# DCMMC/halo2-scaffold

Measured on AMD Instinct MI355X. Metric: create_proof() wall-clock + MSM G1-adds/s at k=20 standard_plonk, 1/2/4/8 GPU, higher is better.
Workload: dtype u32 (254-bit Montgomery integers as 9 x 29-bit limbs, 64-bit multiply-accumulate); 1 GPU; standard_plonk hot-path replay k=20: 11 MSM(2^20) + 6 iNTT(2^20) + 6 coset-NTT(2^21) + 1 coset-iNTT(2^21); k=20, scalar_distribution=uniform, msm_window_bits=17, msm_windows=15, msm_buckets=65536, parallelism=single-gpu, deployment=one process, one GPU, combine=none (single GPU)

## Files before the change

halo2-scaffold_amd/csrc/h2mi_msm.hip:

```cpp

#include <algorithm>
#include <map>
#include <vector>

#include "g1.cuh"
#include "g1_29.cuh"
#include "g1_29_quad.cuh"
#include "h2mi_internal.h"
#include "scan.cuh"

namespace h2 {

constexpr uint32_t S0_MAX = 128;
constexpr uint32_t S1 = 8;
constexpr uint32_t FG_NARROW = 8;
constexpr uint32_t FG_WIDE = 2;
constexpr size_t SHIFT_MIN_N = 4096;
constexpr uint32_t HOT_MIN = 64;
constexpr uint32_t HOT_MIN_WIDE = 8;

constexpr uint32_t ACCUM_RESIDENT_CHUNKS = 256 * 2 * 256;
__host__ __device__ inline uint32_t accum_rounds(uint32_t entries) {
  const uint32_t per_round = S0_MAX * ACCUM_RESIDENT_CHUNKS;
  return entries ? (entries + per_round - 1) / per_round : 1;
}
constexpr uint32_t ACCUM_GATHER_ONLY_MAX = 16384;
__host__ __device__ inline uint32_t accum_chunk_len(uint32_t entries) {
  if (entries <= ACCUM_GATHER_ONLY_MAX) return 1;
  const uint32_t slots = accum_rounds(entries) * ACCUM_RESIDENT_CHUNKS;
  const uint32_t s0 = (entries + slots - 1) / slots;
  return s0 < 8 ? 8 : s0;
}

struct Slot {
  uint32_t* vals[2] = {nullptr, nullptr};
  uint8_t* bkeys = nullptr;
  uint32_t* bincnt = nullptr;
  uint32_t* binbase = nullptr;
  uint32_t* binseg = nullptr;
  uint32_t* tile_live = nullptr;
  uint32_t* off = nullptr;
  uint32_t* s0_dev = nullptr;
  uint32_t* np[2] = {nullptr, nullptr};
  uint32_t* toff[2] = {nullptr, nullptr};
  uint8_t* part[2] = {nullptr, nullptr};
  uint8_t* dense = nullptr;
  uint8_t *dense2 = nullptr, *vsum = nullptr;
  uint32_t* tseg[2] = {nullptr, nullptr};
  uint8_t* rc = nullptr;
  uint8_t* g = nullptr;
  uint64_t* stats = nullptr;
  fe* shift = nullptr;
  hipEvent_t input_ready = nullptr, head_done = nullptr, accum_done = nullptr, tail_done = nullptr;
  bool tail_pending = false, accum_pending = false, head_pending = false;
  bool tail_ever = false, accum_ever = false, head_ever = false;
  hipStream_t last_stream = nullptr;
  bool tail_deferred = false;
  void* d_out = nullptr;
  uint32_t tasks1 = 0;
  uint8_t* sdig = nullptr;
  uint8_t* spart = nullptr;
  uint32_t* scnt = nullptr;
  bool small_deferred = false;
  uint32_t small_n = 0;
};
constexpr int NSLOT = 8;

struct Bases {
  int dev = 0;
  size_t n = 0;
  size_t stride = 0;
  bool has_sum = false;
// ... 95 lines not shown

template <uint32_t CT, class F>
__device__ __forceinline__ void for_each_digit(const fe& s, uint32_t c_rt, uint32_t W_rt, F&& f) {
  const uint32_t c = CT ? CT : c_rt;
  const uint32_t W = CT ? (255 + CT - 1) / CT : W_rt;
  uint32_t carry = 0;
  const uint32_t half = 1u << (c - 1);
#pragma unroll
  for (uint32_t w = 0; w < W; w++) {
    uint32_t bit = w * c;
    uint32_t limb = bit >> 5, sh = bit & 31;
    uint32_t raw = 0;
    if (limb < 8) {
      uint64_t two = s.v[limb];
      if (limb + 1 < 8) two |= (uint64_t)s.v[limb + 1] << 32;
      raw = (uint32_t)(two >> sh) & ((1u << c) - 1);
    }
    uint32_t d = raw + carry;
    uint32_t mag = d, neg = 0;
    carry = 0;
    if (d > half) {
      mag = (1u << c) - d;
      neg = 1;
      carry = 1;
    }
    if (mag) f(w, mag - 1, neg);
  }
}


__device__ __forceinline__ void msm_pick_shift_body(const fe* scalars, size_t n, fe* shift_out) {
  __shared__ fe smp[64];
  const uint32_t lane = threadIdx.x;
  size_t idx = (n / 64) * lane + n / 128;
  if (idx >= n) idx = n - 1;
  const fe v = fe_load(&scalars[idx]);
  smp[lane] = v;
  __syncthreads();
  uint32_t same = 0;
  for (uint32_t j = 0; j < 64; j++) same += fe_eq(v, smp[j]) ? 1u : 0u;
  const uint64_t winners = __ballot(same >= 40);
  if (lane == 0) fe_store(shift_out, winners ? smp[__ffsll((unsigned long long)winners) - 1] : fe_zero());
}
__global__ void __launch_bounds__(64) k_msm_pick_shift(const fe* scalars, size_t n, fe* shift_out) { msm_pick_shift_body(scalars, n, shift_out); }
__device__ __forceinline__ fe msm_scalar(const fe* scalars, size_t i, size_t n, const fe* shift) {
  fe x;
  if (!shift) {
    x = fe_load(&scalars[i]);
  } else {
    const fe v = fe_load(shift);
    x = i < n ? fe_sub<FrP>(fe_load(&scalars[i]), v) : v;
  }
  if (fe_is_zero(x)) return x;
  f29 c = f29_zero();
  c.v[0] = 32;
  fe o;
  f29_pack(f29_reduce_canonical<Fr29>(f29_mul<Fr29>(f29_unpack(x.v), c)), o.v);
  return o;
}

template <uint32_t CT>
__device__ __forceinline__ void msm_bin_count_body(const fe* scalars, size_t n, const fe* shift, uint32_t c, uint32_t W, uint32_t lb, uint32_t nbins,
                                                   uint32_t ntiles, uint32_t* cnt_out, uint32_t* tile_live) {
  __shared__ uint32_t cnt[NBINS_MAX];
  __shared__ uint32_t any_live;
  const uint32_t tid = threadIdx.x;
  if (tid < NBINS_MAX) cnt[tid] = 0;
  if (tid == 0) any_live = 0;
  __syncthreads();
  size_t i = (size_t)blockIdx.x * P1_TS + tid;
  if (i < n + (shift ? 1 : 0)) {
    fe s = msm_scalar(scalars, i, n, shift);
    if (!fe_is_zero(s)) {
      any_live = 1;
      for_each_digit<CT>(s, c, W, [&](uint32_t, uint32_t bucket, uint32_t) { atomicAdd(&cnt[bin_of<(CT >= WIDE_MIN_C)>(bucket, lb)], 1u); });
    }
  }
  __syncthreads();
  if (tid == 0) tile_live[blockIdx.x] = any_live;
  if (tid < nbins) cnt_out[(size_t)tid * ntiles + blockIdx.x] = cnt[tid];
  if (blockIdx.x == 0 && tid == 0) cnt_out[(size_t)nbins * ntiles] = 0;
}
template <uint32_t CT>
__global__ void __launch_bounds__(P1_TS) k_msm_bin_count(const fe* scalars, size_t n, const fe* shift, uint32_t c, uint32_t W, uint32_t lb,
                                                         uint32_t nbins, uint32_t ntiles, uint32_t* cnt_out, uint32_t* tile_live) {
  msm_bin_count_body<CT>(scalars, n, shift, c, W, lb, nbins, ntiles, cnt_out, tile_live);
}

extern __shared__ uint4 h2_msm_smem[];

template <uint32_t CT>
__device__ __forceinline__ void msm_bin_scatter_body(const fe* scalars, size_t n, const fe* shift, size_t n_reg, uint32_t c, uint32_t W, uint32_t lb,
                                                     uint32_t nbins, uint32_t ntiles, const uint32_t* base, uint32_t* vals_out, void* keys_out_,
                                                     const uint32_t* tile_live) {
  constexpr bool WIDE = CT >= WIDE_MIN_C;
  if (!tile_live[blockIdx.x]) return;
  __shared__ uint32_t cnt[NBINS_MAX], lstart[NBINS_MAX + 1], wsum[NBINS_MAX / 64];
  uint32_t* stage_val = reinterpret_cast<uint32_t*>(h2_msm_smem);
  uint16_t* stage_key = reinterpret_cast<uint16_t*>(stage_val + P1_TS * W);
  const uint32_t tid = threadIdx.x, lane = tid & 63, wave = tid >> 6, tile = blockIdx.x;
  uint32_t gb = 0;
  if (tid < NBINS_MAX) {
    cnt[tid] = 0;
    gb = tid < nbins ? base[(size_t)tid * ntiles + tile] : 0;
  }
  __syncthreads();
  size_t i = (size_t)tile * P1_TS + tid;
  fe s;
  const bool live = i < n + (shift ? 1 : 0);
  constexpr uint32_t WK = CT ? (255 + CT - 1) / CT : 1;
  uint32_t ent[WK], rk[WK];
#pragma unroll
  for (uint32_t w = 0; w < WK; w++) ent[w] = 0xFFFFFFFFu;
  bool live_nz = false;
  if (live) {
    s = msm_scalar(scalars, i, n, shift);
    live_nz = !fe_is_zero(s);
  }
  if (live_nz) {
// ... 43 lines not shown
  __syncthreads();
  const uint32_t total = lstart[NBINS_MAX];
  if (WIDE) {
    uint16_t* keys_out = reinterpret_cast<uint16_t*>(keys_out_);
    for (uint32_t p = tid; p < total; p += P1_TS) {
      uint32_t lo = 0, hi = NBINS_MAX;
      while (hi - lo > 1) {
        const uint32_t mid = (lo + hi) >> 1;
        if (lstart[mid] <= p) lo = mid;
        else hi = mid;
      }
      const uint32_t dst = p + cnt[lo];
      vals_out[dst] = stage_val[p];
      keys_out[dst] = stage_key[p];
    }
  } else {
    uint8_t* keys_out = reinterpret_cast<uint8_t*>(keys_out_);
    for (uint32_t p = tid; p < total; p += P1_TS) {
      const uint32_t key = stage_key[p];
      const uint32_t dst = p + cnt[key >> lb];
      vals_out[dst] = stage_val[p];
      keys_out[dst] = (uint8_t)(key & mask);
    }
  }
}
template <uint32_t CT>
__global__ void __launch_bounds__(P1_TS) k_msm_bin_scatter(const fe* scalars, size_t n, const fe* shift, size_t n_reg, uint32_t c, uint32_t W,
                                                           uint32_t lb, uint32_t nbins, uint32_t ntiles, const uint32_t* base, uint32_t* vals_out,
                                                           void* keys_out_, const uint32_t* tile_live) {
  msm_bin_scatter_body<CT>(scalars, n, shift, n_reg, c, W, lb, nbins, ntiles, base, vals_out, keys_out_, tile_live);
}

constexpr uint32_t NQ_MAX = 128;
__device__ __forceinline__ void msm_bin_sort_body(const uint8_t* keys_in, const uint32_t* vals_in, const uint32_t* base, uint32_t ntiles, uint32_t nbins,
                                                  uint32_t lb, uint32_t s0_fixed, uint32_t nb, uint32_t* vals_out, uint32_t* off, uint32_t* np0,
                                                  uint32_t* np1, uint32_t* s0_out) {
  __shared__ uint32_t wh[P2_THREADS / 64][NQ_MAX];
  __shared__ uint32_t run[NQ_MAX], ccnt[NQ_MAX], cstart[NQ_MAX], carry64;
  __shared__ uint32_t stage[P2_CH];
  __shared__ uint8_t stage_q[P2_CH];
  const uint32_t tid = threadIdx.x, wave = tid >> 6, bin = blockIdx.x;
  const uint32_t start = base[(size_t)bin * ntiles], end = base[(size_t)(bin + 1) * ntiles];
  const uint32_t nq = 1u << lb;
  const uint32_t entries = base[(size_t)nbins * ntiles];
  const uint32_t s0 = s0_fixed ? s0_fixed : accum_chunk_len(entries);
  for (uint32_t j = tid; j < (P2_THREADS / 64) * NQ_MAX; j += P2_THREADS) (&wh[0][0])[j] = 0;
  __syncthreads();
  for (uint32_t j = (start & ~15u) + tid * 16; j < end; j += P2_THREADS * 16) {
    const uint4 kk = *reinterpret_cast<const uint4*>(keys_in + j);
    const uint32_t w4[4] = {kk.x, kk.y, kk.z, kk.w};
#pragma unroll
    for (uint32_t t = 0; t < 16; t++) {
      const uint32_t idx = j + t;
      if (idx >= start && idx < end) atomicAdd(&wh[wave][(w4[t >> 2] >> (8 * (t & 3))) & (NQ_MAX - 1)], 1u);
    }
  }
  __syncthreads();
  uint32_t tot = 0, inc = 0;
  if (tid < NQ_MAX) {
#pragma unroll
    for (uint32_t w = 0; w < P2_THREADS / 64; w++) tot += wh[w][tid];
    inc = wave_incl_scan(tot);
    if (tid == 63) carry64 = inc;
  }
  __syncthreads();
  if (tid < NQ_MAX) {
    const uint32_t ex = inc - tot + (tid >= 64 ? carry64 : 0);
    run[tid] = start + ex;
    ccnt[tid] = 0;
    if (tid < nq) {
      const uint32_t b = (bin << lb) + tid;
      const uint32_t o = start + ex;
      off[b] = o;
      uint32_t f0 = tot ? 1u + (o + tot - 1) / s0 - o / s0 : 0u;
      np0[b] = f0;
      np1[b] = (f0 + S1 - 1) / S1;
    }
    if (bin == 0 && tid == 0) {
      off[nb] = entries;
      np0[nb] = 0;
      np1[nb] = 0;
      *s0_out = s0;
    }
  }
  __syncthreads();
  for (uint32_t cs = start; cs < end; cs += P2_CH) {
    const uint32_t m = min(P2_CH, end - cs);
    uint32_t q[P2_PER], v[P2_PER], r[P2_PER];
#pragma unroll
    for (uint32_t k = 0; k < P2_PER; k++) {
      const uint32_t p = k * P2_THREADS + tid;
      if (p < m) {
        q[k] = keys_in[cs + p] & (NQ_MAX - 1);
        v[k] = vals_in[cs + p];
      }
    }
#pragma unroll
    for (uint32_t k = 0; k < P2_PER; k++)
      if (k * P2_THREADS + tid < m) r[k] = atomicAdd(&ccnt[q[k]], 1u);
    __syncthreads();
    uint32_t cn = 0, cinc = 0;
    if (tid < NQ_MAX) {
      cn = ccnt[tid];
      cinc = wave_incl_scan(cn);
      if (tid == 63) carry64 = cinc;
    }
    __syncthreads();
    if (tid < NQ_MAX) cstart[tid] = cinc - cn + (tid >= 64 ? carry64 : 0);
    __syncthreads();
#pragma unroll
    for (uint32_t k = 0; k < P2_PER; k++)
      if (k * P2_THREADS + tid < m) {
        const uint32_t pos = cstart[q[k]] + r[k];
        stage[pos] = v[k];
        stage_q[pos] = (uint8_t)q[k];
      }
    __syncthreads();
    for (uint32_t p = tid; p < m; p += P2_THREADS) {
      const uint32_t qq = stage_q[p];
      vals_out[run[qq] + (p - cstart[qq])] = stage[p];
    }
    __syncthreads();
    if (tid < NQ_MAX) {
      run[tid] += ccnt[tid];
      ccnt[tid] = 0;
    }
    __syncthreads();
  }
}
__global__ void __launch_bounds__(P2_THREADS) k_msm_bin_sort(const uint8_t* keys_in, const uint32_t* vals_in, const uint32_t* base, uint32_t ntiles,
                                                             uint32_t nbins, uint32_t lb, uint32_t s0_fixed, uint32_t nb, uint32_t* vals_out,
                                                             uint32_t* off, uint32_t* np0, uint32_t* np1, uint32_t* s0_out) {
  msm_bin_sort_body(keys_in, vals_in, base, ntiles, nbins, lb, s0_fixed, nb, vals_out, off, np0, np1, s0_out);
}

constexpr uint32_t NQW = 1024, P2W_PER = 12, P2W_CH = P2_THREADS * P2W_PER;
__device__ __forceinline__ void block_excl_scan_1024(const uint32_t* in, uint32_t* out, uint32_t* wtot ) {
  const uint32_t tid = threadIdx.x, lane = tid & 63, wave = tid >> 6;
  const uint32_t a = in[2 * tid], b = in[2 * tid + 1];
  const uint32_t inc = wave_incl_scan(a + b);
  if (lane == 63) wtot[wave] = inc;
  __syncthreads();
  uint32_t add = 0;
  for (uint32_t w = 0; w < wave; w++) add += wtot[w];
  const uint32_t ex = add + inc - (a + b);
  __syncthreads();
  out[2 * tid] = ex;
  out[2 * tid + 1] = ex + a;
}
__global__ void __launch_bounds__(P2_THREADS) k_msm_bin_sort_wide(const uint16_t* keys_in, const uint32_t* vals_in, const uint32_t* base,
                                                                  uint32_t ntiles, uint32_t nbins, uint32_t lb, uint32_t s0_fixed, uint32_t nb,
                                                                  uint32_t* vals_out, uint32_t* off, uint32_t* np0, uint32_t* np1, uint32_t* s0_out) {
  __shared__ uint32_t hist[NQW], run[NQW], ccnt[NQW], cstart[NQW], wtot[P2_THREADS / 64];
  __shared__ uint32_t stage[P2W_CH];
  __shared__ uint16_t stage_q[P2W_CH];
  const uint32_t tid = threadIdx.x, bin = blockIdx.x;
  const uint32_t start = base[(size_t)bin * ntiles], end = base[(size_t)(bin + 1) * ntiles];
  const uint32_t nq = 1u << lb;
  const uint32_t entries = base[(size_t)nbins * ntiles];
  const uint32_t s0 = s0_fixed ? s0_fixed : accum_chunk_len(entries);
  for (uint32_t j = tid; j < NQW; j += P2_THREADS) {
    hist[j] = 0;
    ccnt[j] = 0;
  }
  __syncthreads();
  for (uint32_t j = (start & ~7u) + tid * 8; j < end; j += P2_THREADS * 8) {
// ... 126 lines not shown
      acc = xyzz29_identity();
      do {
        b++;
        bend = off[b + 1];
      } while (bend == k);
    }
    tab_entry p = nxt;
    uint32_t neg = nneg;
    if (k + 1 < end) {
      e = entries[k + 1];
      nxt = tab_load(table, e & 0x7fffffffu);
      nneg = e >> 31;
    }
    if (tab_is_identity(p)) continue;
    f29 x2 = tab_x(p);
    f29 y2 = tab_y(p);
    if (neg) y2 = f29_sub(f29_zero(), y2, Fq29::K2);
    xyzz29_madd(acc, x2, y2);
  }
  part_store(part + (size_t)pidx * PART_BYTES, acc);
}
__global__ void __launch_bounds__(256) k_msm_accum(const uint32_t* entries, const uint32_t* off, const uint32_t* toff, uint32_t nb,
                                                    const uint32_t* s0_dev, const uint8_t* table, uint8_t* part) {
  msm_accum_body(entries, off, toff, nb, s0_dev, table, part);
}

constexpr size_t ACCUM_LDS = 56000;

constexpr uint32_t HEAD_BATCH = 4;
struct HeadDesc {
  const fe* scalars;
  fe* shift;
  uint32_t *bincnt, *tile_live, *binseg, *binbase, *vals0, *vals1, *off, *np0, *np1, *toff0, *toff1, *s0_dev;
  void* bkeys;
  uint8_t* part0;
};
struct HeadBatch {
  HeadDesc d[HEAD_BATCH];
};
__global__ void __launch_bounds__(64) k_msm_pick_shift_b(const HeadBatch hb, size_t n) {
  const HeadDesc& d = hb.d[blockIdx.y];
  msm_pick_shift_body(d.scalars, n, d.shift);
}
template <uint32_t CT>
__global__ void __launch_bounds__(P1_TS) k_msm_bin_count_b(const HeadBatch hb, size_t n, uint32_t c, uint32_t W, uint32_t lb, uint32_t nbins,
                                                           uint32_t ntiles) {
  const HeadDesc& d = hb.d[blockIdx.y];
  msm_bin_count_body<CT>(d.scalars, n, d.shift, c, W, lb, nbins, ntiles, d.bincnt, d.tile_live);
}
template <uint32_t CT>
__global__ void __launch_bounds__(P1_TS) k_msm_bin_scatter_b(const HeadBatch hb, size_t n, size_t n_reg, uint32_t c, uint32_t W, uint32_t lb,
                                                             uint32_t nbins, uint32_t ntiles) {
  const HeadDesc& d = hb.d[blockIdx.y];
  msm_bin_scatter_body<CT>(d.scalars, n, d.shift, n_reg, c, W, lb, nbins, ntiles, d.binbase, d.vals0, d.bkeys, d.tile_live);
}
__global__ void __launch_bounds__(P2_THREADS) k_msm_bin_sort_b(const HeadBatch hb, uint32_t ntiles, uint32_t nbins, uint32_t lb, uint32_t s0_fixed,
                                                               uint32_t nb) {
  const HeadDesc& d = hb.d[blockIdx.y];
  msm_bin_sort_body((const uint8_t*)d.bkeys, d.vals0, d.binbase, ntiles, nbins, lb, s0_fixed, nb, d.vals1, d.off, d.np0, d.np1, d.s0_dev);
}
__global__ void __launch_bounds__(256) k_msm_accum_b(const HeadBatch hb, uint32_t nb, const uint8_t* table) {
  const HeadDesc& d = hb.d[blockIdx.y];
  msm_accum_body(d.vals1, d.off, d.toff0, nb, d.s0_dev, table, d.part0);
}
__global__ void __launch_bounds__(1024) k_scan_segsum_bins_b(const HeadBatch hb, uint32_t m) {
  const HeadDesc& d = hb.d[blockIdx.y];
  scan_segsum_body<SCAN_SEG_BINS>(d.bincnt, m, d.binseg);
}
__global__ void __launch_bounds__(1024) k_scan_seg_bins_b(const HeadBatch hb, uint32_t m) {
  const HeadDesc& d = hb.d[blockIdx.y];
  scan_seg_body<SCAN_SEG_BINS>(d.bincnt, d.binbase, m, d.binseg);
}
__global__ void __launch_bounds__(1024) k_scan_seg_tasks_b(const HeadBatch hb, uint32_t m) {
  const HeadDesc& d = hb.d[blockIdx.z];
  scan_seg_body<SCAN_SEG_TASKS>(blockIdx.y ? d.np1 : d.np0, blockIdx.y ? d.toff1 : d.toff0, m, nullptr);
}

constexpr uint32_t TAIL_BATCH = 8;
struct TailDesc {
  const uint8_t* part0;
  const uint32_t *toff0, *np0, *toff1, *np1, *off;
  uint8_t *part1, *dense, *rc, *g, *out;
  uint64_t* stats;
  uint32_t nb, logNh, logNl, canonical;
  const uint8_t* mat;
  uint8_t *dense2, *vsum;
  uint32_t seg_log;
  uint32_t hot_min;
  uint32_t no_fold;
};
struct TailBatch {
  TailDesc d[TAIL_BATCH];
};

constexpr uint32_t TAIL_THREADS = 512;

template <bool QUAD>
__global__ void __launch_bounds__(256) k_msm_fold(const TailBatch tb) {
  const TailDesc& d = tb.d[blockIdx.y];
  if (d.no_fold) return;
  const uint32_t nb = d.nb;
  const uint32_t *toff_out = d.toff1, *toff_in = d.toff0, *np_in = d.np0;
  const uint32_t t = (blockIdx.x * blockDim.x + threadIdx.x) >> (QUAD ? 2 : 0);
  if (t >= toff_out[nb]) return;
  uint32_t b = find_bucket(toff_out, nb, t);
  uint32_t j = t - toff_out[b];
  const uint32_t m = np_in[b], np = toff_out[b + 1] - toff_out[b];
  const uint32_t q = m / np, r = m - q * np;
// ... 381 lines not shown
  int c = lg >= 22 ? 20 : lg >= 20 ? 17 : lg >= 17 ? 16 : lg >= 11 ? 15 : 13;
  return (uint32_t)c;
}

constexpr size_t SMALL_TABLE_BUDGET = (size_t)2 << 30;
static bool small_geometry(size_t n, uint32_t* c, uint32_t* lanes, uint32_t* r) {
  if (n > SMALL_MAX_N) return false;
  if (getenv("H2MI_MSM_C")) return false;
  uint32_t cc = SMALL_C_MAX;
  while (cc > 2 && ((size_t)1 << (cc - 1)) * ((255 + cc - 1) / cc) * n * 64 > SMALL_TABLE_BUDGET) cc--;
  const size_t cells = n * ((255 + cc - 1) / cc);
  uint32_t ll = SMALL_CELLS, rr = 1;
  if (cells > (size_t)SMALL_CELLS * 256) {
    ll = SMALL_THREADS;
    rr = (uint32_t)((cells + (size_t)SMALL_THREADS * SMALL_PARTS_MAX - 1) / ((size_t)SMALL_THREADS * SMALL_PARTS_MAX));
  }
  *c = cc;
  *lanes = ll;
  *r = rr;
  return true;
}

static uint32_t chunk_override() {
  const char* ev = getenv("H2MI_MSM_S0");
  return (ev && atoi(ev) >= 1 && atoi(ev) <= (int)S0_MAX) ? (uint32_t)atoi(ev) : 0u;
}

static void free_bases(Bases* B) {
  H2_IGNORE(hipFree(B->table));
  H2_IGNORE(hipFree(B->stable));
  H2_IGNORE(hipFree(B->host_stage));
  for (Slot& S : B->slot) {
    H2_IGNORE(hipFree(S.vals[0])); H2_IGNORE(hipFree(S.vals[1]));
    H2_IGNORE(hipFree(S.bkeys)); H2_IGNORE(hipFree(S.bincnt)); H2_IGNORE(hipFree(S.binbase)); H2_IGNORE(hipFree(S.binseg)); H2_IGNORE(hipFree(S.tile_live));
    H2_IGNORE(hipFree(S.off)); H2_IGNORE(hipFree(S.s0_dev));
    for (int i = 0; i < 2; i++) { H2_IGNORE(hipFree(S.np[i])); H2_IGNORE(hipFree(S.toff[i])); }
    H2_IGNORE(hipFree(S.dense)); H2_IGNORE(hipFree(S.dense2)); H2_IGNORE(hipFree(S.vsum)); H2_IGNORE(hipFree(S.tseg[0])); H2_IGNORE(hipFree(S.tseg[1]));
    H2_IGNORE(hipFree(S.part[0])); H2_IGNORE(hipFree(S.part[1])); H2_IGNORE(hipFree(S.rc)); H2_IGNORE(hipFree(S.g)); H2_IGNORE(hipFree(S.stats)); H2_IGNORE(hipFree(S.shift));
    H2_IGNORE(hipFree(S.sdig)); H2_IGNORE(hipFree(S.spart)); H2_IGNORE(hipFree(S.scnt));
    if (S.input_ready) H2_IGNORE(hipEventDestroy(S.input_ready));
    if (S.head_done) H2_IGNORE(hipEventDestroy(S.head_done));
    if (S.accum_done) H2_IGNORE(hipEventDestroy(S.accum_done));
    if (S.tail_done) H2_IGNORE(hipEventDestroy(S.tail_done));
  }
  delete B;
}

#define H2_ALLOC(ptr, bytes)                                   \
  do {                                                         \
    hipError_t e_ = hipMalloc((void**)&(ptr), (bytes));        \
    if (e_ != hipSuccess) {                                    \
      note_hip_error(e_, __FILE__, __LINE__);                  \
      free_bases(B);                                           \
      return e_ == hipErrorOutOfMemory ? H2MI_ENOMEM : H2MI_EHIP; \
    }                                                          \
  } while (0)

static int msm_dev(Bases* B, const void* d_scalars, size_t n, void* d_out, hipStream_t s, bool inorder = false, bool general = false);

static int register_dev(const void* d_bases, size_t n, uint64_t* handle_out, hipStream_t s, bool allow_small = true) {
  if (n == 0 || n > ((size_t)1 << 26)) return H2MI_ERANGE;
  Bases* B = new Bases();
  B->n = n;
  B->dev = ctx().cur;
  B->stride = n + 1;
  B->c = pick_window(n);
  B->W = (255 + B->c - 1) / B->c;
  B->nb = 1u << (B->c - 1);
  B->seg_log = B->c - 1 > MAT_LOG ? B->c - 1 - MAT_LOG : 0;
  B->logNl = (B->c - 1 - B->seg_log + 1) / 2;
  B->logNh = (B->c - 1 - B->seg_log) - B->logNl;
  if ((uint64_t)B->stride * B->W >= (1ull << 31)) { delete B; return H2MI_ERANGE; }
  const size_t nW = B->stride * B->W;
  B->max_tasks0 = std::min(accum_rounds((uint32_t)nW) * ACCUM_RESIDENT_CHUNKS, (uint32_t)nW) + B->nb + 1;
  B->max_tasks1 = B->max_tasks0 / S1 + B->nb;
  H2_ALLOC(B->table, nW * 64);
  B->lb = B->c - 1 > 9 ? B->c - 1 - 9 : 0;
  B->nbins = B->nb >> B->lb;
  const size_t ntiles_max = (B->stride + P1_TS - 1) / P1_TS;
  const size_t bin_cells = (size_t)B->nbins * ntiles_max + 1;
  if (bin_cells >= ((size_t)1 << 31)) { free_bases(B); return H2MI_ERANGE; }
  if ((B->nbins & 3u) || B->nb < 4 || (B->nb > SCAN_SEG_TASKS && !B->seg_log) || B->nbins > NBINS_MAX || (1u << B->lb) > NQW) { free_bases(B); return H2MI_ERANGE; }
  B->nslot = n > ((size_t)1 << 17) ? 4 : NSLOT;
  for (int si_ = 0; si_ < B->nslot; si_++) {
    Slot& S = B->slot[si_];
    for (int i = 0; i < 2; i++) H2_ALLOC(S.vals[i], nW * 4);
    H2_ALLOC(S.bkeys, nW * (B->seg_log ? 2 : 1) + 16);
    H2_ALLOC(S.bincnt, bin_cells * 4);
    H2_ALLOC(S.binbase, bin_cells * 4);
    H2_ALLOC(S.binseg, (bin_cells / SCAN_SEG_BINS + 2) * 4);
    H2_ALLOC(S.tile_live, (ntiles_max + 1) * 4);
    H2_ALLOC(S.off, (size_t)(B->nb + 1) * 4);
    H2_ALLOC(S.s0_dev, 4);
    for (int i = 0; i < 2; i++) {
      H2_ALLOC(S.np[i], (size_t)(B->nb + 1) * 4);
      H2_ALLOC(S.toff[i], (size_t)(B->nb + 1) * 4);
    }
    H2_ALLOC(S.dense, (size_t)B->nb * PART_BYTES);
    if (B->seg_log) {
      H2_ALLOC(S.dense2, ((size_t)1 << MAT_LOG) * PART_BYTES);
      H2_ALLOC(S.vsum, ((size_t)1 << MAT_LOG) * PART_BYTES);
      for (int i = 0; i < 2; i++) H2_ALLOC(S.tseg[i], (size_t)(B->nb / SCAN_SEG_BINS + 2) * 4);
    }
    H2_ALLOC(S.part[0], (size_t)B->max_tasks0 * PART_BYTES);
    H2_ALLOC(S.part[1], (size_t)B->max_tasks1 * PART_BYTES);
    H2_ALLOC(S.rc, (size_t)((2u << B->logNh) + (1u << B->logNl)) * PART_BYTES);
    H2_ALLOC(S.g, (size_t)64 * PART_BYTES);
    H2_ALLOC(S.stats, 64);
    H2_ALLOC(S.shift, 32);
    if (hipEventCreateWithFlags(&S.input_ready, hipEventDisableTiming) != hipSuccess ||
        hipEventCreateWithFlags(&S.head_done, hipEventDisableTiming) != hipSuccess ||
        hipEventCreateWithFlags(&S.accum_done, hipEventDisableTiming) != hipSuccess ||
        hipEventCreateWithFlags(&S.tail_done, hipEventDisableTiming) != hipSuccess) {
      free_bases(B);
      return H2MI_EHIP;
    }
  }
  {
    const bool prof_ = prof_on("k_msm_table_first");
    if (prof_) prof_begin("k_msm_table_first", s);
    hipLaunchKernelGGL(k_msm_table_first, dim3(ceil_div_u32(n, 256)), dim3(256), 0, s, (const uint8_t*)d_bases, B->table, n);
    if (prof_) prof_end(s);
  }
// ... 107 lines not shown
static bool take_small(const Bases* B, bool general) {
  return B->small && !general && !(B->n > SMALL_STREAM_N && B->since_join >= SMALL_STREAM_AFTER);
}
constexpr size_t HEAD_BATCH_MAX_N = (size_t)1 << 17;

static int msm_dev_batch(Bases* B, const void* const* d_scalars, size_t m, size_t n, void* d_out, hipStream_t s, bool inorder) {
  const uint32_t nb = B->nb, W = B->W;
  const bool shifted = B->has_sum && n == B->n;
  const size_t n_eff = n + (shifted ? 1 : 0);
  const uint32_t total = (uint32_t)(n_eff * W);
  hipStream_t hs = inorder ? s : ctx().head_stream, as = hs;
  uint32_t s0_fixed = chunk_override();
  while (s0_fixed && s0_fixed < S0_MAX && ((uint64_t)total + s0_fixed - 1) / s0_fixed + nb > B->max_tasks0) s0_fixed++;
  if (s0_fixed && ((uint64_t)total + s0_fixed - 1) / s0_fixed + nb > B->max_tasks0) return H2MI_ERANGE;
  if ((size_t)P1_TS * W * 6 > 150 * 1024) return H2MI_ERANGE;
  Slot* slots[HEAD_BATCH];
  HeadBatch hb;
  memset(&hb, 0, sizeof(hb));
  for (size_t j = 0; j < m; j++) {
    Slot& S = B->slot[B->next_slot];
    B->last_slot = B->next_slot;
    B->next_slot = (B->next_slot + 1) % B->nslot;
    if (S.tail_deferred) {
      int rc = flush_tails();
      if (rc) return rc;
    }
    if (S.head_pending) H2_HIP(hipStreamWaitEvent(s, S.head_done, 0));
    if (S.tail_pending && S.last_stream != s) H2_HIP(hipStreamWaitEvent(s, S.tail_done, 0));
    S.last_stream = s;
    slots[j] = &S;
    HeadDesc& d = hb.d[j];
    d.scalars = (const fe*)d_scalars[j];
    d.shift = shifted ? S.shift : nullptr;
    d.bincnt = S.bincnt; d.tile_live = S.tile_live; d.binseg = S.binseg; d.binbase = S.binbase;
    d.vals0 = S.vals[0]; d.vals1 = S.vals[1]; d.bkeys = S.bkeys;
    d.off = S.off; d.np0 = S.np[0]; d.np1 = S.np[1]; d.toff0 = S.toff[0]; d.toff1 = S.toff[1]; d.s0_dev = S.s0_dev;
    d.part0 = S.part[0];
  }
  for (size_t j = m; j < HEAD_BATCH; j++) hb.d[j] = hb.d[0];
  const uint32_t ntiles = ceil_div_u32(n_eff, P1_TS), mm = (uint32_t)m;
  static bool attr_set_dev[16] = {};
  bool& attr_set = attr_set_dev[ctx().cur & 15];
  if (!attr_set) {
    H2_HIP(hipFuncSetAttribute(reinterpret_cast<const void*>(k_msm_bin_scatter_b<0>), hipFuncAttributeMaxDynamicSharedMemorySize, 150 * 1024));
    H2_HIP(hipFuncSetAttribute(reinterpret_cast<const void*>(k_msm_bin_scatter_b<13>), hipFuncAttributeMaxDynamicSharedMemorySize, 150 * 1024));
    H2_HIP(hipFuncSetAttribute(reinterpret_cast<const void*>(k_msm_bin_scatter_b<15>), hipFuncAttributeMaxDynamicSharedMemorySize, 150 * 1024));
    H2_HIP(hipFuncSetAttribute(reinterpret_cast<const void*>(k_msm_bin_scatter_b<16>), hipFuncAttributeMaxDynamicSharedMemorySize, 150 * 1024));
    H2_HIP(hipFuncSetAttribute(reinterpret_cast<const void*>(k_msm_bin_scatter_b<17>), hipFuncAttributeMaxDynamicSharedMemorySize, 150 * 1024));
    attr_set = true;
  }
#define H2_BIN_COUNT_B(CT) H2_LAUNCH("k_msm_bin_count", k_msm_bin_count_b<CT>, dim3(ntiles, mm), P1_TS, 0, s, hb, n, B->c, W, B->lb, B->nbins, ntiles)
#define H2_BIN_SCATTER_B(CT) \
  H2_LAUNCH("k_msm_bin_scatter", k_msm_bin_scatter_b<CT>, dim3(ntiles, mm), P1_TS, (size_t)P1_TS * W * 6, s, hb, n, B->stride, B->c, W, B->lb, B->nbins, ntiles)
  if (shifted) H2_LAUNCH("k_msm_pick_shift", k_msm_pick_shift_b, dim3(1, mm), 64, 0, s, hb, n);
  switch (B->c) {
    case 13: H2_BIN_COUNT_B(13); break;
    case 15: H2_BIN_COUNT_B(15); break;
    case 16: H2_BIN_COUNT_B(16); break;
    case 17: H2_BIN_COUNT_B(17); break;
    default: H2_BIN_COUNT_B(0); break;
  }
  const uint32_t cells = B->nbins * ntiles;
  const uint32_t nseg = ceil_div_u32(cells, SCAN_SEG_BINS);
  if (nseg > 1) H2_LAUNCH("k_scan_segsum", k_scan_segsum_bins_b, dim3(nseg, mm), 1024, 0, s, hb, cells);
  H2_LAUNCH("k_scan_seg_bins", k_scan_seg_bins_b, dim3(nseg, mm), 1024, 0, s, hb, cells);
  switch (B->c) {
    case 13: H2_BIN_SCATTER_B(13); break;
    case 15: H2_BIN_SCATTER_B(15); break;
    case 16: H2_BIN_SCATTER_B(16); break;
    case 17: H2_BIN_SCATTER_B(17); break;
    default: H2_BIN_SCATTER_B(0); break;
  }
#undef H2_BIN_COUNT_B
#undef H2_BIN_SCATTER_B
  if (hs != s) {
    H2_HIP(hipEventRecord(slots[0]->input_ready, s));
    H2_HIP(hipStreamWaitEvent(hs, slots[0]->input_ready, 0));
  }
  for (size_t j = 0; j < m; j++) {
    Slot& S = *slots[j];
    if (S.accum_pending) H2_HIP(hipStreamWaitEvent(hs, S.accum_done, 0));
    if (S.tail_pending) H2_HIP(hipStreamWaitEvent(hs, S.tail_done, 0));
    S.tail_pending = S.accum_pending = S.head_pending = false;
  }
  H2_LAUNCH("k_msm_bin_sort", k_msm_bin_sort_b, dim3(B->nbins, mm), P2_THREADS, 0, hs, hb, ntiles, B->nbins, B->lb, s0_fixed, nb);
  H2_LAUNCH("k_scan_seg_tasks", k_scan_seg_tasks_b, dim3(1, 2, mm), 1024, 0, hs, hb, nb);
  const uint32_t chunks0 = s0_fixed ? (uint32_t)(((uint64_t)total + s0_fixed - 1) / s0_fixed) : std::min(accum_rounds(total) * ACCUM_RESIDENT_CHUNKS, total);
  const uint32_t tasks0 = chunks0 + nb;
  for (size_t j = 0; j < m; j++) {
    H2_HIP(hipEventRecord(slots[j]->head_done, hs));
    slots[j]->head_pending = true;
    slots[j]->head_ever = true;
  }
  if (as != hs) H2_HIP(hipStreamWaitEvent(as, slots[m - 1]->head_done, 0));
  H2_LAUNCH("k_msm_accum", k_msm_accum_b, dim3(ceil_div_u32(chunks0, 256), mm), 256, ACCUM_LDS, as, hb, nb, (const uint8_t*)B->table);
  for (size_t j = 0; j < m; j++) {
    Slot& S = *slots[j];
    S.d_out = (char*)d_out + 96 * j;
    S.tasks1 = tasks0 / S1 + nb;
    H2_HIP(hipEventRecord(S.accum_done, as));
    S.accum_pending = true;
    S.accum_ever = true;
    if (!inorder) {
      S.tail_deferred = true;
      g_deferred.push_back({B, &S});
    }
  }
  if (inorder) {
    TailBatch tb;
    for (size_t j = 0; j < m; j++) tb.d[j] = tail_desc(B, *slots[j]);
    for (size_t j = m; j < TAIL_BATCH; j++) tb.d[j] = tb.d[0];
    int rc = launch_tails(tb, mm, slots[0]->tasks1, nb, B->logNh, B->logNl, B->seg_log, s);
    if (rc) return rc;
    for (size_t j = 0; j < m; j++) {
      Slot& S = *slots[j];
      H2_HIP(hipEventRecord(S.tail_done, s));
      S.tail_pending = true;
      S.tail_ever = true;
    }
// ... 80 lines not shown
  hipStream_t hs = s, as = s;
  uint32_t s0_fixed = chunk_override();
  while (s0_fixed && s0_fixed < S0_MAX && ((uint64_t)total + s0_fixed - 1) / s0_fixed + nb > B->max_tasks0) s0_fixed++;
  if (s0_fixed && ((uint64_t)total + s0_fixed - 1) / s0_fixed + nb > B->max_tasks0) return H2MI_ERANGE;
  if (pipelined) {
    hs = ctx().head_stream;
    as = ctx().accum_stream;
    if (S.head_pending) H2_HIP(hipStreamWaitEvent(s, S.head_done, 0));
    if (S.tail_pending && S.last_stream != s) H2_HIP(hipStreamWaitEvent(s, S.tail_done, 0));
  } else {
    if (S.head_ever) H2_HIP(hipStreamWaitEvent(s, S.head_done, 0));
    if (S.accum_ever) H2_HIP(hipStreamWaitEvent(s, S.accum_done, 0));
    if (S.tail_ever) H2_HIP(hipStreamWaitEvent(s, S.tail_done, 0));
  }
  S.last_stream = s;
  const uint32_t ntiles = ceil_div_u32(n_eff, P1_TS);
  const fe* shift = shifted ? S.shift : nullptr;
  static bool attr_set_dev[16] = {};
  bool& attr_set = attr_set_dev[ctx().cur & 15];
  if ((size_t)P1_TS * W * 6 > 150 * 1024) return H2MI_ERANGE;
  if (!attr_set) {
    H2_HIP(hipFuncSetAttribute(reinterpret_cast<const void*>(k_msm_bin_scatter<0>), hipFuncAttributeMaxDynamicSharedMemorySize, 150 * 1024));
    H2_HIP(hipFuncSetAttribute(reinterpret_cast<const void*>(k_msm_bin_scatter<13>), hipFuncAttributeMaxDynamicSharedMemorySize, 150 * 1024));
    H2_HIP(hipFuncSetAttribute(reinterpret_cast<const void*>(k_msm_bin_scatter<15>), hipFuncAttributeMaxDynamicSharedMemorySize, 150 * 1024));
    H2_HIP(hipFuncSetAttribute(reinterpret_cast<const void*>(k_msm_bin_scatter<16>), hipFuncAttributeMaxDynamicSharedMemorySize, 150 * 1024));
    H2_HIP(hipFuncSetAttribute(reinterpret_cast<const void*>(k_msm_bin_scatter<17>), hipFuncAttributeMaxDynamicSharedMemorySize, 150 * 1024));
    H2_HIP(hipFuncSetAttribute(reinterpret_cast<const void*>(k_msm_bin_scatter<18>), hipFuncAttributeMaxDynamicSharedMemorySize, 150 * 1024));
    H2_HIP(hipFuncSetAttribute(reinterpret_cast<const void*>(k_msm_bin_scatter<19>), hipFuncAttributeMaxDynamicSharedMemorySize, 150 * 1024));
    H2_HIP(hipFuncSetAttribute(reinterpret_cast<const void*>(k_msm_bin_scatter<20>), hipFuncAttributeMaxDynamicSharedMemorySize, 150 * 1024));
    attr_set = true;
  }
  {
#define H2_BIN_COUNT(CT) \
  H2_LAUNCH("k_msm_bin_count", k_msm_bin_count<CT>, ntiles, P1_TS, 0, s, (const fe*)d_scalars, n, shift, B->c, W, B->lb, B->nbins, ntiles, S.bincnt, S.tile_live)
#define H2_BIN_SCATTER(CT)                                                                                                                        \
  H2_LAUNCH("k_msm_bin_scatter", k_msm_bin_scatter<CT>, ntiles, P1_TS, (size_t)P1_TS * W * 6, s, (const fe*)d_scalars, n, shift, B->stride, B->c, W, \
            B->lb, B->nbins, ntiles, (const uint32_t*)S.binbase, S.vals[0], S.bkeys, (const uint32_t*)S.tile_live)
    if (shifted) H2_LAUNCH("k_msm_pick_shift", k_msm_pick_shift, 1, 64, 0, s, (const fe*)d_scalars, n, S.shift);
    switch (B->c) {
      case 13: H2_BIN_COUNT(13); break;
      case 15: H2_BIN_COUNT(15); break;
      case 16: H2_BIN_COUNT(16); break;
      case 17: H2_BIN_COUNT(17); break;
      case 18: H2_BIN_COUNT(18); break;
      case 19: H2_BIN_COUNT(19); break;
      case 20: H2_BIN_COUNT(20); break;
      default: H2_BIN_COUNT(0); break;
    }
    const uint32_t cells = B->nbins * ntiles;
    const uint32_t nseg = ceil_div_u32(cells, SCAN_SEG_BINS);
    if (nseg > 1) H2_LAUNCH("k_scan_segsum", k_scan_segsum<SCAN_SEG_BINS>, nseg, 1024, 0, s, (const uint32_t*)S.bincnt, cells, S.binseg);
    H2_LAUNCH("k_scan_seg_bins", k_scan_seg<SCAN_SEG_BINS>, dim3(nseg, 1), 1024, 0, s, (const uint32_t*)S.bincnt, S.binbase, (const uint32_t*)nullptr,
              (uint32_t*)nullptr, cells, (const uint32_t*)S.binseg);
    switch (B->c) {
      case 13: H2_BIN_SCATTER(13); break;
      case 15: H2_BIN_SCATTER(15); break;
      case 16: H2_BIN_SCATTER(16); break;
      case 17: H2_BIN_SCATTER(17); break;
      case 18: H2_BIN_SCATTER(18); break;
      case 19: H2_BIN_SCATTER(19); break;
      case 20: H2_BIN_SCATTER(20); break;
      default: H2_BIN_SCATTER(0); break;
    }
#undef H2_BIN_COUNT
#undef H2_BIN_SCATTER
  }
  if (pipelined) {
    H2_HIP(hipEventRecord(S.input_ready, s));
    H2_HIP(hipStreamWaitEvent(hs, S.input_ready, 0));
    if (S.accum_pending) H2_HIP(hipStreamWaitEvent(hs, S.accum_done, 0));
    if (S.tail_pending) H2_HIP(hipStreamWaitEvent(hs, S.tail_done, 0));
  }
  S.tail_pending = false;
  S.accum_pending = false;
  S.head_pending = false;
  if (B->seg_log) {
    H2_LAUNCH("k_msm_bin_sort", k_msm_bin_sort_wide, B->nbins, P2_THREADS, 0, hs, (const uint16_t*)S.bkeys, (const uint32_t*)S.vals[0],
              (const uint32_t*)S.binbase, ntiles, B->nbins, B->lb, s0_fixed, nb, S.vals[1], S.off, S.np[0], S.np[1], S.s0_dev);
    const uint32_t tsegs = ceil_div_u32(nb, SCAN_SEG_BINS);
    for (int i = 0; i < 2; i++) {
      H2_LAUNCH("k_scan_segsum", k_scan_segsum<SCAN_SEG_BINS>, tsegs, 1024, 0, hs, (const uint32_t*)S.np[i], nb, S.tseg[i]);
      H2_LAUNCH("k_scan_seg_tasks", k_scan_seg<SCAN_SEG_BINS>, dim3(tsegs, 1), 1024, 0, hs, (const uint32_t*)S.np[i], S.toff[i], (const uint32_t*)nullptr,
                (uint32_t*)nullptr, nb, (const uint32_t*)S.tseg[i]);
    }
  } else {
    H2_LAUNCH("k_msm_bin_sort", k_msm_bin_sort, B->nbins, P2_THREADS, 0, hs, (const uint8_t*)S.bkeys, (const uint32_t*)S.vals[0],
              (const uint32_t*)S.binbase, ntiles, B->nbins, B->lb, s0_fixed, nb, S.vals[1], S.off, S.np[0], S.np[1], S.s0_dev);
    H2_LAUNCH("k_scan_seg_tasks", k_scan_seg<SCAN_SEG_TASKS>, dim3(1, 2), 1024, 0, hs, (const uint32_t*)S.np[0], S.toff[0], (const uint32_t*)S.np[1], S.toff[1], nb,
              (const uint32_t*)nullptr);
  }
  const uint32_t chunks0 = s0_fixed ? (uint32_t)(((uint64_t)total + s0_fixed - 1) / s0_fixed) : std::min(accum_rounds(total) * ACCUM_RESIDENT_CHUNKS, total);
  const uint32_t tasks0 = chunks0 + nb;
  if (pipelined) {
    H2_HIP(hipEventRecord(S.head_done, hs));
    H2_HIP(hipStreamWaitEvent(as, S.head_done, 0));
    S.head_pending = true;
    S.head_ever = true;
  }
  H2_LAUNCH("k_msm_accum", k_msm_accum, ceil_div_u32(chunks0, 256), 256, ACCUM_LDS, as, (const uint32_t*)S.vals[1], (const uint32_t*)S.off,
            (const uint32_t*)S.toff[0], nb, (const uint32_t*)S.s0_dev, (const uint8_t*)B->table, S.part[0]);
  S.d_out = d_out;
  S.tasks1 = tasks0 / S1 + nb;
  if (pipelined) {
    H2_HIP(hipEventRecord(S.accum_done, as));
    S.accum_pending = true;
    S.accum_ever = true;
    S.tail_deferred = true;
    g_deferred.push_back({B, &S});
    if (g_deferred.size() >= (size_t)std::max(1, B->nslot / 2)) return flush_tails();
    return H2MI_OK;
  }
  TailBatch tb;
  for (uint32_t j = 0; j < TAIL_BATCH; j++) tb.d[j] = tail_desc(B, S);
  int rc = launch_tails(tb, 1, S.tasks1, nb, B->logNh, B->logNl, B->seg_log, s);
  if (rc) return rc;
  H2_HIP(hipEventRecord(S.tail_done, s));
  S.tail_pending = true;
  S.tail_ever = true;
  return H2MI_OK;
}

static SmallDesc small_desc(const Bases* B, const Slot& S) {
// ... 651 lines not shown
```

Baseline: 9.465 billion G1-adds/s.

## Fuse shift pick into bin count and task-offset scan into bin sort via decoupled lookback

Removes the separate pick-shift kernel: every bin-count block now recomputes the shift sample into shared memory, and block 0 writes it out. Removes the separate task-offset scan kernel by having each bin-sort block publish its per-bin task-count aggregate and compute an exclusive prefix through a decoupled lookback over a new per-slot binlb array. The aim is fewer kernel launches and serial dependencies on the MSM head path. In exchange every count block does extra redundant scalar loads and compares, and correctness now depends on bin-sort blocks making forward progress and on binlb being reset in the count kernel before each sort.

```diff
diff --git a/halo2-scaffold_amd/csrc/h2mi_msm.hip b/halo2-scaffold_amd/csrc/h2mi_msm.hip
--- a/halo2-scaffold_amd/csrc/h2mi_msm.hip
+++ b/halo2-scaffold_amd/csrc/h2mi_msm.hip
@@ -38,6 +38,7 @@
   uint32_t* bincnt = nullptr;
   uint32_t* binbase = nullptr;
   uint32_t* binseg = nullptr;
+  uint64_t* binlb = nullptr;
   uint32_t* tile_live = nullptr;
   uint32_t* off = nullptr;
   uint32_t* s0_dev = nullptr;
@@ -199,17 +200,21 @@
 __device__ __forceinline__ void msm_pick_shift_body(const fe* scalars, size_t n, fe* shift_out) {
   __shared__ fe smp[64];
   const uint32_t lane = threadIdx.x;
-  size_t idx = (n / 64) * lane + n / 128;
-  if (idx >= n) idx = n - 1;
-  const fe v = fe_load(&scalars[idx]);
-  smp[lane] = v;
-  __syncthreads();
-  uint32_t same = 0;
-  for (uint32_t j = 0; j < 64; j++) same += fe_eq(v, smp[j]) ? 1u : 0u;
-  const uint64_t winners = __ballot(same >= 40);
-  if (lane == 0) fe_store(shift_out, winners ? smp[__ffsll((unsigned long long)winners) - 1] : fe_zero());
-}
-__global__ void __launch_bounds__(64) k_msm_pick_shift(const fe* scalars, size_t n, fe* shift_out) { msm_pick_shift_body(scalars, n, shift_out); }
+  fe v;
+  if (lane < 64) {
+    size_t idx = (n / 64) * lane + n / 128;
+    if (idx >= n) idx = n - 1;
+    v = fe_load(&scalars[idx]);
+    smp[lane] = v;
+  }
+  __syncthreads();
+  if (lane < 64) {
+    uint32_t same = 0;
+    for (uint32_t j = 0; j < 64; j++) same += fe_eq(v, smp[j]) ? 1u : 0u;
+    const uint64_t winners = __ballot(same >= 40);
+    if (lane == 0) fe_store(shift_out, winners ? smp[__ffsll((unsigned long long)winners) - 1] : fe_zero());
+  }
+}
 __device__ __forceinline__ fe msm_scalar(const fe* scalars, size_t i, size_t n, const fe* shift) {
   fe x;
   if (!shift) {
@@ -227,17 +232,21 @@
 }
 
 template <uint32_t CT>
-__device__ __forceinline__ void msm_bin_count_body(const fe* scalars, size_t n, const fe* shift, uint32_t c, uint32_t W, uint32_t lb, uint32_t nbins,
-                                                   uint32_t ntiles, uint32_t* cnt_out, uint32_t* tile_live) {
+__device__ __forceinline__ void msm_bin_count_body(const fe* scalars, size_t n, fe* shift, uint32_t c, uint32_t W, uint32_t lb, uint32_t nbins,
+                                                   uint32_t ntiles, uint32_t* cnt_out, uint32_t* tile_live, uint64_t* binlb) {
   __shared__ uint32_t cnt[NBINS_MAX];
   __shared__ uint32_t any_live;
+  __shared__ __align__(16) fe shift_sh;
   const uint32_t tid = threadIdx.x;
   if (tid < NBINS_MAX) cnt[tid] = 0;
   if (tid == 0) any_live = 0;
-  __syncthreads();
+  if (blockIdx.x == 0 && tid < NBINS_MAX) binlb[tid] = 0;
+  if (shift) msm_pick_shift_body(scalars, n, &shift_sh);
+  __syncthreads();
+  if (shift && blockIdx.x == 0 && tid == 0) fe_store(shift, shift_sh);
   size_t i = (size_t)blockIdx.x * P1_TS + tid;
   if (i < n + (shift ? 1 : 0)) {
-    fe s = msm_scalar(scalars, i, n, shift);
+    fe s = msm_scalar(scalars, i, n, shift ? &shift_sh : nullptr);
     if (!fe_is_zero(s)) {
       any_live = 1;
       for_each_digit<CT>(s, c, W, [&](uint32_t, uint32_t bucket, uint32_t) { atomicAdd(&cnt[bin_of<(CT >= WIDE_MIN_C)>(bucket, lb)], 1u); });
@@ -249,9 +258,9 @@
   if (blockIdx.x == 0 && tid == 0) cnt_out[(size_t)nbins * ntiles] = 0;
 }
 template <uint32_t CT>
-__global__ void __launch_bounds__(P1_TS) k_msm_bin_count(const fe* scalars, size_t n, const fe* shift, uint32_t c, uint32_t W, uint32_t lb,
-                                                         uint32_t nbins, uint32_t ntiles, uint32_t* cnt_out, uint32_t* tile_live) {
-  msm_bin_count_body<CT>(scalars, n, shift, c, W, lb, nbins, ntiles, cnt_out, tile_live);
+__global__ void __launch_bounds__(P1_TS) k_msm_bin_count(const fe* scalars, size_t n, fe* shift, uint32_t c, uint32_t W, uint32_t lb, uint32_t nbins,
+                                                         uint32_t ntiles, uint32_t* cnt_out, uint32_t* tile_live, uint64_t* binlb) {
+  msm_bin_count_body<CT>(scalars, n, shift, c, W, lb, nbins, ntiles, cnt_out, tile_live, binlb);
 }
 
 extern __shared__ uint4 h2_msm_smem[];
@@ -361,11 +370,43 @@
 }
 
 constexpr uint32_t NQ_MAX = 128;
+
+constexpr uint64_t LB_AGG = 1ull << 62, LB_INCL = 2ull << 62;
+typedef __attribute__((address_space(1))) uint64_t lb_word;
+__device__ __forceinline__ void lb_publish(uint64_t* w, uint64_t tag, uint32_t t0, uint32_t t1) {
+  __hip_atomic_store((lb_word*)w, tag | ((uint64_t)t1 << 31) | t0, __ATOMIC_RELAXED, __HIP_MEMORY_SCOPE_AGENT);
+}
+__device__ __forceinline__ void lb_prefix(uint64_t* lbw, uint32_t bin, uint32_t& p0, uint32_t& p1) {
+  const uint32_t lane = threadIdx.x & 63;
+  uint32_t a0 = 0, a1 = 0;
+  int j = (int)bin;
+  while (j > 0) {
+    const int idx = j - 1 - (int)lane;
+    const uint64_t v = idx >= 0 ? __hip_atomic_load((lb_word*)(lbw + idx), __ATOMIC_RELAXED, __HIP_MEMORY_SCOPE_AGENT) : LB_INCL;
+    const uint64_t tag = v & (3ull << 62);
+    const uint64_t notyet = __ballot(tag == 0), incl = __ballot(tag == LB_INCL);
+    const uint32_t fn = notyet ? (uint32_t)__ffsll((unsigned long long)notyet) - 1 : 64u;
+    const uint32_t fi = incl ? (uint32_t)__ffsll((unsigned long long)incl) - 1 : 64u;
+    const uint32_t take = fn < fi ? fn : (fi < 64 ? fi + 1 : 64u);
+    if (lane < take) {
+      a0 += (uint32_t)(v & 0x7FFFFFFFu);
+      a1 += (uint32_t)((v >> 31) & 0x7FFFFFFFu);
+    }
+    if (fi < fn) break;
+    j -= (int)take;
+    if (!take) __builtin_amdgcn_s_sleep(2);
+  }
+  a0 = wave_incl_scan(a0);
+  a1 = wave_incl_scan(a1);
+  p0 = __shfl(a0, 63);
+  p1 = __shfl(a1, 63);
+}
+
 __device__ __forceinline__ void msm_bin_sort_body(const uint8_t* keys_in, const uint32_t* vals_in, const uint32_t* base, uint32_t ntiles, uint32_t nbins,
                                                   uint32_t lb, uint32_t s0_fixed, uint32_t nb, uint32_t* vals_out, uint32_t* off, uint32_t* np0,
-                                                  uint32_t* np1, uint32_t* s0_out) {
+                                                  uint32_t* np1, uint32_t* toff0, uint32_t* toff1, uint64_t* binlb, uint32_t* s0_out) {
   __shared__ uint32_t wh[P2_THREADS / 64][NQ_MAX];
-  __shared__ uint32_t run[NQ_MAX], ccnt[NQ_MAX], cstart[NQ_MAX], carry64;
+  __shared__ uint32_t run[NQ_MAX], ccnt[NQ_MAX], cstart[NQ_MAX], carry64, tcarry[2], tagg[2], tpre[2];
   __shared__ uint32_t stage[P2_CH];
   __shared__ uint8_t stage_q[P2_CH];
   const uint32_t tid = threadIdx.x, wave = tid >> 6, bin = blockIdx.x;
@@ -385,7 +426,7 @@
     }
   }
   __syncthreads();
-  uint32_t tot = 0, inc = 0;
+  uint32_t tot = 0, inc = 0, f0 = 0, f1 = 0, i0 = 0, i1 = 0;
   if (tid < NQ_MAX) {
 #pragma unroll
     for (uint32_t w = 0; w < P2_THREADS / 64; w++) tot += wh[w][tid];
@@ -401,9 +442,10 @@
       const uint32_t b = (bin << lb) + tid;
       const uint32_t o = start + ex;
       off[b] = o;
-      uint32_t f0 = tot ? 1u + (o + tot - 1) / s0 - o / s0 : 0u;
+      f0 = tot ? 1u + (o + tot - 1) / s0 - o / s0 : 0u;
+      f1 = (f0 + S1 - 1) / S1;
       np0[b] = f0;
-      np1[b] = (f0 + S1 - 1) / S1;
+      np1[b] = f1;
     }
     if (bin == 0 && tid == 0) {
       off[nb] = entries;
@@ -411,8 +453,23 @@
       np1[nb] = 0;
       *s0_out = s0;
     }
-  }
-  __syncthreads();
+    i0 = wave_incl_scan(f0);
+    i1 = wave_incl_scan(f1);
+    if (tid == 63) {
+      tcarry[0] = i0;
+      tcarry[1] = i1;
+    }
+  }
+  __syncthreads();
+  if (tid >= 64 && tid < NQ_MAX) {
+    i0 += tcarry[0];
+    i1 += tcarry[1];
+    if (tid == NQ_MAX - 1) {
+      tagg[0] = i0;
+      tagg[1] = i1;
+      lb_publish(binlb + bin, bin ? LB_AGG : LB_INCL, i0, i1);
+    }
+  }
   for (uint32_t cs = start; cs < end; cs += P2_CH) {
     const uint32_t m = min(P2_CH, end - cs);
     uint32_t q[P2_PER], v[P2_PER], r[P2_PER];
@@ -456,11 +513,32 @@
     }
     __syncthreads();
   }
+  __syncthreads();
+  if (tid < 64) {
+    uint32_t p0 = 0, p1 = 0;
+    if (bin) lb_prefix(binlb, bin, p0, p1);
+    if (tid == 0) {
+      tpre[0] = p0;
+      tpre[1] = p1;
+      if (bin) lb_publish(binlb + bin, LB_INCL, p0 + tagg[0], p1 + tagg[1]);
+    }
+  }
+  __syncthreads();
+  if (tid < nq) {
+    const uint32_t b = (bin << lb) + tid;
+    toff0[b] = tpre[0] + i0 - f0;
+    toff1[b] = tpre[1] + i1 - f1;
+  }
+  if (bin == nbins - 1 && tid == NQ_MAX - 1) {
+    toff0[nb] = tpre[0] + i0;
+    toff1[nb] = tpre[1] + i1;
+  }
 }
 __global__ void __launch_bounds__(P2_THREADS) k_msm_bin_sort(const uint8_t* keys_in, const uint32_t* vals_in, const uint32_t* base, uint32_t ntiles,
                                                              uint32_t nbins, uint32_t lb, uint32_t s0_fixed, uint32_t nb, uint32_t* vals_out,
-                                                             uint32_t* off, uint32_t* np0, uint32_t* np1, uint32_t* s0_out) {
-  msm_bin_sort_body(keys_in, vals_in, base, ntiles, nbins, lb, s0_fixed, nb, vals_out, off, np0, np1, s0_out);
+                                                             uint32_t* off, uint32_t* np0, uint32_t* np1, uint32_t* toff0, uint32_t* toff1,
+                                                             uint64_t* binlb, uint32_t* s0_out) {
+  msm_bin_sort_body(keys_in, vals_in, base, ntiles, nbins, lb, s0_fixed, nb, vals_out, off, np0, np1, toff0, toff1, binlb, s0_out);
 }
 
 constexpr uint32_t NQW = 1024, P2W_PER = 12, P2W_CH = P2_THREADS * P2W_PER;
@@ -653,21 +731,18 @@
   const fe* scalars;
   fe* shift;
   uint32_t *bincnt, *tile_live, *binseg, *binbase, *vals0, *vals1, *off, *np0, *np1, *toff0, *toff1, *s0_dev;
+  uint64_t* binlb;
   void* bkeys;
   uint8_t* part0;
 };
 struct HeadBatch {
   HeadDesc d[HEAD_BATCH];
 };
-__global__ void __launch_bounds__(64) k_msm_pick_shift_b(const HeadBatch hb, size_t n) {
-  const HeadDesc& d = hb.d[blockIdx.y];
-  msm_pick_shift_body(d.scalars, n, d.shift);
-}
 template <uint32_t CT>
 __global__ void __launch_bounds__(P1_TS) k_msm_bin_count_b(const HeadBatch hb, size_t n, uint32_t c, uint32_t W, uint32_t lb, uint32_t nbins,
                                                            uint32_t ntiles) {
   const HeadDesc& d = hb.d[blockIdx.y];
-  msm_bin_count_body<CT>(d.scalars, n, d.shift, c, W, lb, nbins, ntiles, d.bincnt, d.tile_live);
+  msm_bin_count_body<CT>(d.scalars, n, d.shift, c, W, lb, nbins, ntiles, d.bincnt, d.tile_live, d.binlb);
 }
 template <uint32_t CT>
 __global__ void __launch_bounds__(P1_TS) k_msm_bin_scatter_b(const HeadBatch hb, size_t n, size_t n_reg, uint32_t c, uint32_t W, uint32_t lb,
@@ -678,7 +753,8 @@
 __global__ void __launch_bounds__(P2_THREADS) k_msm_bin_sort_b(const HeadBatch hb, uint32_t ntiles, uint32_t nbins, uint32_t lb, uint32_t s0_fixed,
                                                                uint32_t nb) {
   const HeadDesc& d = hb.d[blockIdx.y];
-  msm_bin_sort_body((const uint8_t*)d.bkeys, d.vals0, d.binbase, ntiles, nbins, lb, s0_fixed, nb, d.vals1, d.off, d.np0, d.np1, d.s0_dev);
+  msm_bin_sort_body((const uint8_t*)d.bkeys, d.vals0, d.binbase, ntiles, nbins, lb, s0_fixed, nb, d.vals1, d.off, d.np0, d.np1, d.toff0, d.toff1, d.binlb,
+                    d.s0_dev);
 }
 __global__ void __launch_bounds__(256) k_msm_accum_b(const HeadBatch hb, uint32_t nb, const uint8_t* table) {
   const HeadDesc& d = hb.d[blockIdx.y];
@@ -691,10 +767,6 @@
 __global__ void __launch_bounds__(1024) k_scan_seg_bins_b(const HeadBatch hb, uint32_t m) {
   const HeadDesc& d = hb.d[blockIdx.y];
   scan_seg_body<SCAN_SEG_BINS>(d.bincnt, d.binbase, m, d.binseg);
-}
-__global__ void __launch_bounds__(1024) k_scan_seg_tasks_b(const HeadBatch hb, uint32_t m) {
-  const HeadDesc& d = hb.d[blockIdx.z];
-  scan_seg_body<SCAN_SEG_TASKS>(blockIdx.y ? d.np1 : d.np0, blockIdx.y ? d.toff1 : d.toff0, m, nullptr);
 }
 
 constexpr uint32_t TAIL_BATCH = 8;
@@ -1142,7 +1214,7 @@
   H2_IGNORE(hipFree(B->host_stage));
   for (Slot& S : B->slot) {
     H2_IGNORE(hipFree(S.vals[0])); H2_IGNORE(hipFree(S.vals[1]));
-    H2_IGNORE(hipFree(S.bkeys)); H2_IGNORE(hipFree(S.bincnt)); H2_IGNORE(hipFree(S.binbase)); H2_IGNORE(hipFree(S.binseg)); H2_IGNORE(hipFree(S.tile_live));
+    H2_IGNORE(hipFree(S.bkeys)); H2_IGNORE(hipFree(S.bincnt)); H2_IGNORE(hipFree(S.binbase)); H2_IGNORE(hipFree(S.binseg)); H2_IGNORE(hipFree(S.binlb)); H2_IGNORE(hipFree(S.tile_live));
     H2_IGNORE(hipFree(S.off)); H2_IGNORE(hipFree(S.s0_dev));
     for (int i = 0; i < 2; i++) { H2_IGNORE(hipFree(S.np[i])); H2_IGNORE(hipFree(S.toff[i])); }
     H2_IGNORE(hipFree(S.dense)); H2_IGNORE(hipFree(S.dense2)); H2_IGNORE(hipFree(S.vsum)); H2_IGNORE(hipFree(S.tseg[0])); H2_IGNORE(hipFree(S.tseg[1]));
@@ -1190,7 +1262,7 @@
   const size_t ntiles_max = (B->stride + P1_TS - 1) / P1_TS;
   const size_t bin_cells = (size_t)B->nbins * ntiles_max + 1;
   if (bin_cells >= ((size_t)1 << 31)) { free_bases(B); return H2MI_ERANGE; }
-  if ((B->nbins & 3u) || B->nb < 4 || (B->nb > SCAN_SEG_TASKS && !B->seg_log) || B->nbins > NBINS_MAX || (1u << B->lb) > NQW) { free_bases(B); return H2MI_ERANGE; }
+  if ((B->nbins & 3u) || B->nb < 4 || (B->nb > NBINS_MAX * NQ_MAX && !B->seg_log) || B->nbins > NBINS_MAX || (1u << B->lb) > NQW) { free_bases(B); return H2MI_ERANGE; }
   B->nslot = n > ((size_t)1 << 17) ? 4 : NSLOT;
   for (int si_ = 0; si_ < B->nslot; si_++) {
     Slot& S = B->slot[si_];
@@ -1199,6 +1271,7 @@
     H2_ALLOC(S.bincnt, bin_cells * 4);
     H2_ALLOC(S.binbase, bin_cells * 4);
     H2_ALLOC(S.binseg, (bin_cells / SCAN_SEG_BINS + 2) * 4);
+    H2_ALLOC(S.binlb, NBINS_MAX * 8);
     H2_ALLOC(S.tile_live, (ntiles_max + 1) * 4);
     H2_ALLOC(S.off, (size_t)(B->nb + 1) * 4);
     H2_ALLOC(S.s0_dev, 4);
@@ -1372,7 +1445,7 @@
     HeadDesc& d = hb.d[j];
     d.scalars = (const fe*)d_scalars[j];
     d.shift = shifted ? S.shift : nullptr;
-    d.bincnt = S.bincnt; d.tile_live = S.tile_live; d.binseg = S.binseg; d.binbase = S.binbase;
+    d.bincnt = S.bincnt; d.tile_live = S.tile_live; d.binseg = S.binseg; d.binbase = S.binbase; d.binlb = S.binlb;
     d.vals0 = S.vals[0]; d.vals1 = S.vals[1]; d.bkeys = S.bkeys;
     d.off = S.off; d.np0 = S.np[0]; d.np1 = S.np[1]; d.toff0 = S.toff[0]; d.toff1 = S.toff[1]; d.s0_dev = S.s0_dev;
     d.part0 = S.part[0];
@@ -1392,7 +1465,6 @@
 #define H2_BIN_COUNT_B(CT) H2_LAUNCH("k_msm_bin_count", k_msm_bin_count_b<CT>, dim3(ntiles, mm), P1_TS, 0, s, hb, n, B->c, W, B->lb, B->nbins, ntiles)
 #define H2_BIN_SCATTER_B(CT) \
   H2_LAUNCH("k_msm_bin_scatter", k_msm_bin_scatter_b<CT>, dim3(ntiles, mm), P1_TS, (size_t)P1_TS * W * 6, s, hb, n, B->stride, B->c, W, B->lb, B->nbins, ntiles)
-  if (shifted) H2_LAUNCH("k_msm_pick_shift", k_msm_pick_shift_b, dim3(1, mm), 64, 0, s, hb, n);
   switch (B->c) {
     case 13: H2_BIN_COUNT_B(13); break;
     case 15: H2_BIN_COUNT_B(15); break;
@@ -1424,7 +1496,6 @@
     S.tail_pending = S.accum_pending = S.head_pending = false;
   }
   H2_LAUNCH("k_msm_bin_sort", k_msm_bin_sort_b, dim3(B->nbins, mm), P2_THREADS, 0, hs, hb, ntiles, B->nbins, B->lb, s0_fixed, nb);
-  H2_LAUNCH("k_scan_seg_tasks", k_scan_seg_tasks_b, dim3(1, 2, mm), 1024, 0, hs, hb, nb);
   const uint32_t chunks0 = s0_fixed ? (uint32_t)(((uint64_t)total + s0_fixed - 1) / s0_fixed) : std::min(accum_rounds(total) * ACCUM_RESIDENT_CHUNKS, total);
   const uint32_t tasks0 = chunks0 + nb;
   for (size_t j = 0; j < m; j++) {
@@ -1571,11 +1642,11 @@
   }
   {
 #define H2_BIN_COUNT(CT) \
-  H2_LAUNCH("k_msm_bin_count", k_msm_bin_count<CT>, ntiles, P1_TS, 0, s, (const fe*)d_scalars, n, shift, B->c, W, B->lb, B->nbins, ntiles, S.bincnt, S.tile_live)
+  H2_LAUNCH("k_msm_bin_count", k_msm_bin_count<CT>, ntiles, P1_TS, 0, s, (const fe*)d_scalars, n, shifted ? S.shift : nullptr, B->c, W, B->lb, \
+            B->nbins, ntiles, S.bincnt, S.tile_live, S.binlb)
 #define H2_BIN_SCATTER(CT)                                                                                                                        \
   H2_LAUNCH("k_msm_bin_scatter", k_msm_bin_scatter<CT>, ntiles, P1_TS, (size_t)P1_TS * W * 6, s, (const fe*)d_scalars, n, shift, B->stride, B->c, W, \
             B->lb, B->nbins, ntiles, (const uint32_t*)S.binbase, S.vals[0], S.bkeys, (const uint32_t*)S.tile_live)
-    if (shifted) H2_LAUNCH("k_msm_pick_shift", k_msm_pick_shift, 1, 64, 0, s, (const fe*)d_scalars, n, S.shift);
     switch (B->c) {
       case 13: H2_BIN_COUNT(13); break;
       case 15: H2_BIN_COUNT(15); break;
@@ -1624,9 +1695,8 @@
     }
   } else {
     H2_LAUNCH("k_msm_bin_sort", k_msm_bin_sort, B->nbins, P2_THREADS, 0, hs, (const uint8_t*)S.bkeys, (const uint32_t*)S.vals[0],
-              (const uint32_t*)S.binbase, ntiles, B->nbins, B->lb, s0_fixed, nb, S.vals[1], S.off, S.np[0], S.np[1], S.s0_dev);
-    H2_LAUNCH("k_scan_seg_tasks", k_scan_seg<SCAN_SEG_TASKS>, dim3(1, 2), 1024, 0, hs, (const uint32_t*)S.np[0], S.toff[0], (const uint32_t*)S.np[1], S.toff[1], nb,
-              (const uint32_t*)nullptr);
+              (const uint32_t*)S.binbase, ntiles, B->nbins, B->lb, s0_fixed, nb, S.vals[1], S.off, S.np[0], S.np[1], S.toff[0], S.toff[1], S.binlb,
+              S.s0_dev);
   }
   const uint32_t chunks0 = s0_fixed ? (uint32_t)(((uint64_t)total + s0_fixed - 1) / s0_fixed) : std::min(accum_rounds(total) * ACCUM_RESIDENT_CHUNKS, total);
   const uint32_t tasks0 = chunks0 + nb;
```

Result: no change. 9.372 billion G1-adds/s (median of 2 runs) (-1.0%).
